# ComparativeGenomicsToolkit/cactus

Measured on NVIDIA B200. Metric: BAR POA DP Gcells/sec and ends/sec at 1/2/4/8 B200 vs reference CPU BAR, higher is better.
Workload: dtype int32

## Files before the change

cactus_b200/csrc/poa_cta.cuh:

```cuda
#pragma once
#include <cuda_runtime.h>
#include "poa_graph.cuh"

namespace barb200 {

__device__ int cta_excl_scan(int *a, int n, int *ws) {
    const int T = blockDim.x, tid = threadIdx.x, lane = tid & 31, warp = tid >> 5, nw = T >> 5;
    const int chunk = (n + T - 1) / T, b = min(n, tid * chunk), e = min(n, b + chunk);
    int s = 0;
    for (int i = b; i < e; ++i) s += a[i];
    int inc = s;
#pragma unroll
    for (int off = 1; off < 32; off <<= 1) { const int v = __shfl_up_sync(0xffffffffu, inc, off); if (lane >= off) inc += v; }
    __syncthreads();
    if (lane == 31) ws[warp] = inc;
    __syncthreads();
    int woff = 0, total = 0;
    for (int k = 0; k < nw; ++k) { const int v = ws[k]; if (k < warp) woff += v; total += v; }
    int run = woff + inc - s;
    for (int i = b; i < e; ++i) { const int v = a[i]; a[i] = run; run += v; }
    __syncthreads();
    return total;
}

// ... 99 lines not shown
    if (first_new + n_new > g.node_cap) { if (tid == 0) g.err = JOB_ERR_NODE_CAP; __syncthreads(); return; }
    for (int q = tid; q < L; q += T) {
        const int m = node_of[q];
        if (m >= 0) { is_new[q] = 0; continue; }
        const int nid = first_new + is_new[q];
        g.base[nid] = seq[q]; g.aln_n[nid] = 0;
        g.in_off[nid] = 0; g.in_n[nid] = 0; g.in_cap[nid] = 0; g.out_off[nid] = 0; g.out_n[nid] = 0; g.out_cap[nid] = 0;
        if (m != INT32_MIN) graph_add_aligned(g, -1 - m, nid);
        node_of[q] = nid; is_new[q] = 1;
    }
    if (tid == 0) g.node_n = first_new + n_new;
    __syncthreads();
    if (g.err) return;
    {
        int *anc = g.remain, *cnt = g.msa_rank, *new_i2n = g.tmp1;
        const int n_old = first_new;
        for (int q = tid; q < L; q += T) {
            const int v = node_of[q];
            int e = v < first_new ? g.node_to_index[v] : -1;
            for (int k = 0; k < g.aln_n[v]; ++k) { const int a = g.aln_id[v * 4 + k]; if (a < first_new) e = max(e, g.node_to_index[a]); }
            anc[q] = e;
        }
        for (int i = tid; i < n_old; i += T) cnt[i] = 0;
        __syncthreads();
        cta_incl_max_scan(anc, L, ws);
        for (int q = tid; q < L; q += T) if (node_of[q] >= first_new) atomicAdd(&cnt[max(anc[q], 0)], 1);
        __syncthreads();
        cta_excl_scan(cnt, n_old, ws);
        for (int i = tid; i < n_old; i += T) new_i2n[i + cnt[i]] = g.index_to_node[i];
        for (int q = tid; q < L; q += T) { const int v = node_of[q]; if (v >= first_new) new_i2n[max(anc[q], 0) + 1 + (v - first_new)] = v; }
        __syncthreads();
        for (int k = tid; k < first_new + n_new; k += T) { const int v = new_i2n[k]; g.index_to_node[k] = v; g.node_to_index[v] = k; }
        __syncthreads();
    }
    for (int q = tid; q <= L; q += T) {
        const int from = q == 0 ? SRC_ID : node_of[q - 1], to = q == L ? SINK_ID : node_of[q];
        const int fresh = (q > 0 && from >= first_new) || (q < L && to >= first_new);
        graph_add_edge_par(g, from, to, fresh ? 0 : 1, read_id);
    }
    __syncthreads();
}


__device__ __forceinline__ void prefetch_l2(const void *p) { asm volatile("prefetch.global.L2 [%0];" ::"l"(p)); }

__device__ int warp_backtrack_step(const RowTables &rt, const DpState &d, const PoaParams &P, const int *smat8, const uint8_t *q,
                                   int &i, int &j, int &cur_op, int &len) {
    const unsigned FULLM = 0xffffffffu;
    const int lane = threadIdx.x & 31, inf = P.inf_min, e1 = P.e1, e2 = P.e2, oe1 = P.o1 + P.e1, oe2 = P.o2 + P.e2;
    len = 1;
    const RowRec rc = rt.rec[i];
    const RowInfo ri = d.info[i];
    const int *rowi = d.planes + d.row_off[i];
    const int npre = rc.base_npre >> 8;
    const int s = smat8[8 * (rc.base_npre & 0xff) + q[j - 1]];
    int hij = inf; unsigned cij = (unsigned)E_NEG16 | (unsigned)E_NEG16 << 16;
    if (j >= ri.beg && j <= ri.end) { const int64_t o = plane_index(ri.beg, ri.end, 0, j); hij = __ldcg(rowi + o); cij = (unsigned)__ldcg(rowi + o + CPT); }
    int hk0 = inf;
    if ((cur_op & OP_F) && j - 1 - lane >= ri.beg && j - 1 - lane <= ri.end) hk0 = __ldcg(rowi + plane_index(ri.beg, ri.end, 0, j - 1 - lane));
    int pi = -1, pm = inf, ph = inf, pe1 = inf, pe2 = inf; bool m_in = false, e_in = false;
    auto probe = [&](int kb) {
        const int k = kb + lane;
        pi = -1; m_in = false; e_in = false;
        if (k >= npre) return;
        pi = k == 0 ? rc.pre0 : rt.pre_row[rc.pre_off + k];
        const RowInfo pin = d.info[pi];
        const int *prow = d.planes + d.row_off[pi];
        m_in = (cur_op & OP_M) && j - 1 >= pin.beg && j - 1 <= pin.end;
        e_in = (cur_op & OP_E) && j >= pin.beg && j <= pin.end;
        if (m_in) pm = __ldcg(prow + plane_index(pin.beg, pin.end, 0, j - 1));
        if (e_in) {
            const int64_t o = plane_index(pin.beg, pin.end, 0, j);
            ph = __ldcg(prow + o);
            const unsigned code = (unsigned)__ldcg(prow + o + CPT);
            pe1 = e_decode(ph, (int)(code & 0xffffu), inf); pe2 = e_decode(ph, (int)(code >> 16), inf);
        }
    };
    if (cur_op & OP_M) {
        for (int kb = 0; kb < npre; kb += 32) {
            probe(kb);
            const unsigned hit = __ballot_sync(FULLM, m_in && pm + s == hij);
            if (hit) { i = __shfl_sync(FULLM, pi, __ffs(hit) - 1); --j; cur_op = OP_ALL; return CMATCH; }
        }
    }
    if (cur_op & OP_E) {
        const int own_e1 = e_decode(hij, (int)(cij & 0xffffu), inf), own_e2 = e_decode(hij, (int)(cij >> 16), inf);
        for (int kb = 0; kb < npre; kb += 32) {
            if (npre > 32 || !(cur_op & OP_M)) probe(kb);
            const bool ok1 = e_in && (cur_op & OP_E1) && ((cur_op & OP_M) ? hij == pe1 : own_e1 == pe1 - e1);
            const bool ok2 = e_in && (cur_op & OP_E2) && ((cur_op & OP_M) ? hij == pe2 : own_e2 == pe2 - e2);
            const unsigned hit = __ballot_sync(FULLM, ok1 || ok2);
            if (hit) {
                const int f = __ffs(hit) - 1;
                const int nop = ok1 ? ((ph - oe1 == pe1) ? (OP_M | OP_F) : OP_E1) : ((ph - oe2 == pe2) ? (OP_M | OP_F) : OP_E2);
                cur_op = __shfl_sync(FULLM, nop, f); i = __shfl_sync(FULLM, pi, f);
                return CDEL;
            }
        }
    }
    if (cur_op & OP_F) {
        if (!(cur_op & OP_M)) return -1;
        const int avail = j - ri.beg;
        int t1_max;
        if (e1 > e2) t1_max = oe2 >= oe1 ? (oe2 - oe1) / (e1 - e2) + 1 : 0;
        else t1_max = (e1 < e2 || oe1 <= oe2) ? avail : 0;
        if (t1_max > avail) t1_max = avail;
        for (int which = 0; which < 2; ++which) {
            if (!(cur_op & (which ? OP_F2 : OP_F1))) continue;
            const int oe = which ? oe2 : oe1, e = which ? e2 : e1, tmax = which ? avail : t1_max;
            for (int t0 = 0; t0 < tmax; t0 += 32) {
                const int t = t0 + lane + 1;
                int hk = hk0;
                if (t0 > 0) { hk = inf; if (t <= avail) hk = __ldcg(rowi + plane_index(ri.beg, ri.end, 0, j - t)); }
                const unsigned hit = __ballot_sync(FULLM, t <= tmax && hk == hij + oe + (t - 1) * e);
                if (hit) { len = __ffs(hit); len += t0; j -= len; cur_op = OP_M | OP_E; return CINS; }
            }
        }
    }
    return -1;
}

__device__ void warp_backtrack(Graph &g, const RowTables &rt, DpState &d, const PoaParams &P, const int *smat8, const uint8_t *q, int L) {
    const unsigned FULLM = 0xffffffffu;
    const int lane = threadIdx.x & 31, inf = P.inf_min;
    if (lane == 0) { dp_best_cell(g, rt, d, P, L); d.fc_row = -1; d.fc_hi = -1; }
    __syncwarp();
    int i = d.best_i, j = d.best_j, cur_op = OP_ALL, nc = 0, last_op = -1;
    uint64_t *cg = d.cigar; const int cap = d.cigar_cap;
    int fail = 0;
    auto push = [&](int op, int len, int node_id, int query_id) {
        if (nc == 0 || op != CINS || last_op != CINS) {
            if (nc >= cap) { fail = JOB_ERR_CIGAR_CAP; return; }
            if (lane == 0) {
                const uint64_t n_id = (uint64_t)(int64_t)node_id, q_id = (uint64_t)(int64_t)query_id, l = (uint64_t)len;
                cg[nc] = op == CMATCH ? (n_id << 34 | q_id << 4 | (uint64_t)op) : op == CINS ? (q_id << 34 | l << 4 | (uint64_t)op) : (n_id << 34 | l << 4 | (uint64_t)op);
            }
            ++nc;
        } else if (lane == 0) cg[nc - 1] += (uint64_t)len << 4;
        last_op = op;
    };
    if (j < L) push(CINS, L - j, -1, L - 1);
#ifdef BT_PROFILE
    long long pf_t0 = clock64(), pf_run_t = 0, pf_step_t = 0; int pf_iters = 0, pf_runs = 0, pf_cells = 0, pf_steps = 0, pf_ins = 0;
#endif
    while (i > 0 && j > 0 && !fail) {
        int run = 0;
#ifdef BT_PROFILE
        long long pf_a = clock64();
#endif
        if (cur_op == OP_ALL) {
            int c = i - lane, pre = -1, base = 0, n_ok = 0, node = 0;
            RowInfo ric; ric.beg = 0; ric.end = -1; ric.left = 0; ric.right = 0;
            int64_t ro = 0;
            bool fresh = true;
#pragma unroll 1
            for (int it = 0; it < 4; ++it) {
                if (fresh) {
                    pre = -1;
                    if (c > 0) { const RowRec rc = rt.rec[c]; base = rc.base_npre & 0xff; pre = (rc.base_npre >> 8) ? rc.pre0 : -1; node = g.index_to_node[c]; }
                    if (c >= 0) { ric = d.info[c]; ro = d.row_off[c]; }
                }
                const int nxt = __shfl_down_sync(FULLM, c, 1);
                const bool ok = lane < 31 && pre >= 0 && pre == nxt;
                n_ok = __ffs(~__ballot_sync(FULLM, ok)) - 1;
                if (n_ok >= 31 || it == 3) break;
                const int pre_b = __shfl_sync(FULLM, pre, n_ok);
                if (pre_b < 0) break;
                fresh = lane > n_ok;
                if (fresh) c = pre_b - (lane - n_ok - 1);
            }
            const int jj = j - lane;
            int hv = inf, inb = 0;
            if (lane <= n_ok && c >= 0 && jj >= 0) {
                inb = jj >= ric.beg && jj <= ric.end;
                if (inb) hv = __ldcg(d.planes + ro + plane_index(ric.beg, ric.end, 0, jj));
            }
            const int cl = c - 32, jl = jj - 32;
            RowInfo ril; ril.beg = 0; ril.end = -1; ril.left = 0; ril.right = 0;
            int64_t rol = 0;
            if (cl >= 0 && jl >= 0) { ril = d.info[cl]; rol = d.row_off[cl]; prefetch_l2(rt.rec + cl); prefetch_l2(g.index_to_node + cl); }
            const int h_next = __shfl_down_sync(FULLM, hv, 1), inb_next = __shfl_down_sync(FULLM, inb, 1);
            bool hit = false;
            if (lane < n_ok && c > 0 && jj >= 1 && inb_next) hit = h_next + smat8[8 * base + q[jj - 1]] == hv;
            run = __ffs(~__ballot_sync(FULLM, hit)) - 1;
            if (run > 0) {
                if (nc + run > cap) fail = JOB_ERR_CIGAR_CAP;
                else {
                    if (lane < run) cg[nc + lane] = (uint64_t)node << 34 | (uint64_t)(jj - 1) << 4 | (uint64_t)CMATCH;
                    nc += run; last_op = CMATCH;
                    i = __shfl_sync(FULLM, c, run); j -= run;
                }
            }
            if (cl >= 0 && jl >= 0 && jl <= ril.end) prefetch_l2(d.planes + rol + plane_index(ril.beg, ril.end, 0, jl < ril.beg ? ril.beg : jl));
        }
#ifdef BT_PROFILE
        long long pf_b = clock64(); if (cur_op == OP_ALL) { pf_run_t += pf_b - pf_a; ++pf_iters; if (run) { ++pf_runs; pf_cells += run; } }
#endif
        if (run == 0 && !fail) {
            const int id = g.index_to_node[i], jq = j - 1;
            int len = 1;
            const int op = warp_backtrack_step(rt, d, P, smat8, q, i, j, cur_op, len);
            if (op < 0) fail = JOB_ERR_BACKTRACK; else push(op, len, id, jq);
#ifdef BT_PROFILE
            pf_step_t += clock64() - pf_b; ++pf_steps; if (op == CINS) ++pf_ins;
#endif
        }
    }
#ifdef BT_PROFILE
    if (lane == 0 && blockIdx.x == 0) printf("bt L=%d total=%lld run_t=%lld step_t=%lld iters=%d runs=%d cells=%d steps=%d ins=%d\n", L, clock64() - pf_t0, pf_run_t, pf_step_t, pf_iters, pf_runs, pf_cells, pf_steps, pf_ins);
#endif
    if (!fail && j > 0) push(CINS, j, -1, j - 1);
    if (fail) { if (lane == 0) g.err = fail; return; }
// ... 173 lines not shown
```

cactus_b200/csrc/poa_graph.cuh:

```cuda
#pragma once
#include <stdio.h>
#include "poa_types.h"

namespace barb200 {

HD void graph_reset(Graph &g, int n_seq) {
    g.node_n = 2; g.W = 1 + ((n_seq - 1) >> 6);
    g.in_used = 0; g.out_used = 0; g.err = JOB_OK;
    for (int i = 0; i < 2; ++i) {
        g.base[i] = 0; g.aln_n[i] = 0;
        g.in_off[i] = 0; g.in_n[i] = 0; g.in_cap[i] = 0;
        g.out_off[i] = 0; g.out_n[i] = 0; g.out_cap[i] = 0;
    }
}

HD int graph_add_node(Graph &g, uint8_t b) {
    if (g.node_n >= g.node_cap) { g.err = JOB_ERR_NODE_CAP; return g.node_cap - 1; }
    int id = g.node_n++;
    g.base[id] = b; g.aln_n[id] = 0;
    g.in_off[id] = 0; g.in_n[id] = 0; g.in_cap[id] = 0;
    g.out_off[id] = 0; g.out_n[id] = 0; g.out_cap[id] = 0;
    return id;
}

// ... 81 lines not shown
    g.err = JOB_ERR_TOPO;
}

HD void graph_sort_node_edges(Graph &g, int v) {
    {
        const int o = g.in_off[v], n = g.in_n[v];
        for (int j = 0; j < n - 1; ++j) for (int k = j + 1; k < n; ++k)
            if (g.in_w[o + j] < g.in_w[o + k]) {
                int t = g.in_id[o + j]; g.in_id[o + j] = g.in_id[o + k]; g.in_id[o + k] = t;
                t = g.in_w[o + j]; g.in_w[o + j] = g.in_w[o + k]; g.in_w[o + k] = t;
            }
    }
    {
        const int o = g.out_off[v], n = g.out_n[v], W = g.W;
        for (int j = 0; j < n - 1; ++j) for (int k = j + 1; k < n; ++k)
            if (g.out_w[o + j] < g.out_w[o + k]) {
                int t = g.out_id[o + j]; g.out_id[o + j] = g.out_id[o + k]; g.out_id[o + k] = t;
                t = g.out_w[o + j]; g.out_w[o + j] = g.out_w[o + k]; g.out_w[o + k] = t;
                for (int w = 0; w < W; ++w) {
                    uint64_t r = g.out_rid[(int64_t)(o + j) * W + w];
                    g.out_rid[(int64_t)(o + j) * W + w] = g.out_rid[(int64_t)(o + k) * W + w];
                    g.out_rid[(int64_t)(o + k) * W + w] = r;
                }
            }
    }
}

HD void graph_bfs_remain(Graph &g) {
    const int n = g.node_n;
    int *outdeg = g.tmp0, *q = g.tmp1;
    for (int i = 0; i < n; ++i) { outdeg[i] = g.out_n[i]; g.remain[i] = 0; }
    int head = 0, tail = 0;
    q[tail++] = SINK_ID; g.remain[SINK_ID] = -1;
    while (head < tail) {
        const int cur = q[head++];
        if (cur != SINK_ID) {
            int max_w = -1, max_id = -1;
            const int oo = g.out_off[cur], on = g.out_n[cur];
            for (int i = 0; i < on; ++i) if (g.out_w[oo + i] > max_w) { max_w = g.out_w[oo + i]; max_id = g.out_id[oo + i]; }
            g.remain[cur] = g.remain[max_id] + 1;
        }
        if (cur == SRC_ID) return;
        const int io = g.in_off[cur], in = g.in_n[cur];
        for (int i = 0; i < in; ++i) if (--outdeg[g.in_id[io + i]] == 0) q[tail++] = g.in_id[io + i];
    }
    g.err = JOB_ERR_TOPO;
}

HD void graph_build_row(const Graph &g, RowTables &rt, int r, int off) {
    const int v = g.index_to_node[r];
    const int io = g.in_off[v], in = g.in_n[v];
    for (int k = 0; k < in; ++k) rt.pre_row[off + k] = g.node_to_index[g.in_id[io + k]];
    RowRec rec;
    rec.base_npre = g.base[v] | (in << 8);
    rec.rd = g.remain[v] - g.remain[SINK_ID] - 1;
    rec.pre_off = off;
    rec.pre0 = in ? g.node_to_index[g.in_id[io]] : -1;
    rt.rec[r] = rec;
}
HD void graph_build_rows(const Graph &g, RowTables &rt) {
    int off = 0;
    for (int r = 0; r < g.node_n; ++r) { graph_build_row(g, rt, r, off); off += g.in_n[g.index_to_node[r]]; }
}
HD int row_npre(const RowTables &rt, int r) { return rt.rec[r].base_npre >> 8; }
HD int row_base(const RowTables &rt, int r) { return rt.rec[r].base_npre & 0xff; }

HD void graph_topo_sort_serial(Graph &g, RowTables &rt) {
    graph_bfs_index(g);
    if (g.err) return;
    for (int v = 0; v < g.node_n; ++v) graph_sort_node_edges(g, v);
    graph_bfs_remain(g);
    if (g.err) return;
    graph_build_rows(g, rt);
}

HD void graph_add_first_sequence(Graph &g, const uint8_t *seq, int len, int read_id) {
    int last = SRC_ID;
    for (int i = 0; i < len; ++i) { int cur = graph_add_node(g, seq[i]); graph_add_edge(g, last, cur, 0, read_id); last = cur; if (g.err) return; }
    graph_add_edge(g, last, SINK_ID, 0, read_id);
}

HD void graph_fuse_alignment(Graph &g, const uint8_t *seq, const uint64_t *cigar, int n_cigar, int read_id) {
    if (n_cigar == 0) return;
    int query_id = -1, last_new = 0, last_id = SRC_ID;
    for (int i = 0; i < n_cigar && !g.err; ++i) {
        const int op = (int)(cigar[i] & 0xf);
        if (op == CMATCH) {
            const int node_id = (int)((cigar[i] >> 34) & 0x3fffffff);
            ++query_id;
            const uint8_t b = seq[query_id];
            if (g.base[node_id] != b) {
                int a = graph_aligned_with_base(g, node_id, b);
                if (a != -1) { graph_add_edge(g, last_id, a, 1 - last_new, read_id); last_id = a; last_new = 0; }
                else {
                    int nid = graph_add_node(g, b);
                    graph_add_edge(g, last_id, nid, 0, read_id);
                    last_id = nid; last_new = 1;
                    graph_add_aligned(g, node_id, nid);
                }
            } else { graph_add_edge(g, last_id, node_id, 1 - last_new, read_id); last_id = node_id; last_new = 0; }
        } else if (op == CINS) {
            const int len = (int)((cigar[i] >> 4) & 0x3fffffff);
            query_id += len;
            for (int j = len - 1; j >= 0 && !g.err; --j) {
                int nid = graph_add_node(g, seq[query_id - j]);
                graph_add_edge(g, last_id, nid, 0, read_id);
                last_id = nid; last_new = 1;
            }
        }
    }
    if (!g.err) graph_add_edge(g, last_id, SINK_ID, 1 - last_new, read_id);
}

HD int graph_msa_rank(Graph &g) {
    const int n = g.node_n;
    int *indeg = g.tmp0, *st = g.tmp1;
    for (int i = 0; i < n; ++i) indeg[i] = g.in_n[i];
    int sp = 0, rank = 0;
// ... 250 lines not shown
```

cactus_b200/csrc/poa_kernel.cu:

```cuda
#include <cuda_runtime.h>
#include <stdint.h>
#include "poa_graph.cuh"
#include "poa_cta.cuh"
#include "poa_kernel.cuh"

namespace barb200 {

#define FULL 0xffffffffu

struct KShared {
    Graph g; RowTables rt; DpState d;
    int job, msa_len_s, abort_s;
    int smat[5 * 8];
    int wF[2][2][32];
    int wM[2][4][32];
};

__device__ __forceinline__ int4 ld4cg(const int *p) { return __ldcg(reinterpret_cast<const int4 *>(p)); }
__device__ __forceinline__ void st4(int *p, int a, int b, int c, int d) { *reinterpret_cast<int4 *>(p) = make_int4(a, b, c, d); }
__device__ __forceinline__ int max3(int a, int b, int c) { return max(max(a, b), c); }
__device__ __forceinline__ void st8(int *p, int a0, int a1, int a2, int a3, int a4, int a5, int a6, int a7) {
    asm volatile("st.global.v8.b32 [%0], {%1,%2,%3,%4,%5,%6,%7,%8};" ::"l"(p), "r"(a0), "r"(a1), "r"(a2), "r"(a3), "r"(a4), "r"(a5), "r"(a6), "r"(a7) : "memory");
}
struct int8v { int v[8]; };
__device__ __forceinline__ int8v ld8cg(const int *p) {
    int8v r;
    asm volatile("ld.global.cg.v8.b32 {%0,%1,%2,%3,%4,%5,%6,%7}, [%8];" : "=r"(r.v[0]), "=r"(r.v[1]), "=r"(r.v[2]), "=r"(r.v[3]), "=r"(r.v[4]), "=r"(r.v[5]), "=r"(r.v[6]), "=r"(r.v[7]) : "l"(p) : "memory");
    return r;
}


template <bool MASKED>
__device__ __forceinline__ void row_pass1(int (&H)[CPT], int (&E1)[CPT], int (&E2)[CPT], const int *mrow, const uint32_t (&qc)[2],
                                          int j0, int beg, int end, int NEG, int je1, int je2, int e1, int e2, int &agg1, int &agg2) {
#pragma unroll
    for (int e = 0; e < CPT; ++e) {
        const int s = mrow[(qc[e >> 3] >> ((e & 7) * 4)) & 7];
        int h = __vimax3_s32(H[e] + s, E1[e], E2[e]);
        if (MASKED) {
            const bool inb = (unsigned)(j0 + e - beg) <= (unsigned)(end - beg);
            h = inb ? h : NEG; E1[e] = inb ? E1[e] : NEG; E2[e] = inb ? E2[e] : NEG;
        }
        H[e] = h;
        agg1 = __viaddmax_s32(h, je1 + e * e1, agg1); agg2 = __viaddmax_s32(h, je2 + e * e2, agg2);
    }
}

template <int MODE>
__device__ __forceinline__ void row_pass2(int (&H)[CPT], int (&E1)[CPT], int (&E2)[CPT], int P1, int P2, int j0, int beg, int end, int NEG,
                                          int je1, int je2, int e1, int e2, int o1, int o2, int *tp, int &tmax) {
    const int oe1 = o1 + e1, oe2 = o2 + e2;
#pragma unroll
    for (int oc = 0; oc < 2; ++oc) {
        int dd[8];
#pragma unroll
        for (int u = 0; u < 8; ++u) {
            const int e = oc * 8 + u, u1 = je1 + e * e1, u2 = je2 + e * e2;
            const int f1 = P1 - o1 - u1, f2 = P2 - o2 - u2;
            P1 = __viaddmax_s32(H[e], u1, P1); P2 = __viaddmax_s32(H[e], u2, P2);
            int h = __vimax3_s32(H[e], f1, f2);
            int x1 = __viaddmax_s32(E1[e], -e1, h - oe1);
            int x2 = __viaddmax_s32(E2[e], -e2, h - oe2);
            if (MODE == 1) {
                const bool inb = (unsigned)(j0 + e - beg) <= (unsigned)(end - beg);
                h = inb ? h : NEG; x1 = inb ? x1 : NEG; x2 = inb ? x2 : NEG;
            } else if (MODE == 2) {
                const bool inb = j0 + e <= end;
                h = inb ? h : NEG; x1 = inb ? x1 : NEG; x2 = inb ? x2 : NEG;
            }
            H[e] = h; E1[e] = x1; E2[e] = x2;
            dd[u] = (h - x1) | ((h - x2) << 16);
            tmax = max(tmax, h);
        }
        st8(tp + CPT + oc * 8, dd[0], dd[1], dd[2], dd[3], dd[4], dd[5], dd[6], dd[7]);
    }
#pragma unroll
    for (int oc = 0; oc < 2; ++oc)
        st8(tp + oc * 8, H[oc * 8], H[oc * 8 + 1], H[oc * 8 + 2], H[oc * 8 + 3], H[oc * 8 + 4], H[oc * 8 + 5], H[oc * 8 + 6], H[oc * 8 + 7]);
}

template <bool MASKED>
__device__ __forceinline__ void row_argmax(const int (&H)[CPT], int v, int j0, int beg, int end, int &tl, int &tr) {
    unsigned m = 0;
#pragma unroll
    for (int e = 0; e < CPT; ++e) m |= H[e] == v ? 1u << e : 0u;
    if (MASKED) {
        const int lo = max(beg - j0, 0), hi = min(end - j0, CPT - 1);
        m &= (2u << hi) - (1u << lo);
    }
    if (m) { tl = j0 + __ffs(m) - 1; tr = j0 + 31 - __clz(m); }
}

__device__ long long dp_sweep(KShared &S, const BatchArgs &A, const uint8_t *__restrict__ qg, int L) {
    const int tid = threadIdx.x, lane = tid & 31, warp = tid >> 5, nwarps = blockDim.x >> 5;
    const PoaParams &P = A.P;
    uint8_t *const sb = A.slots + (int64_t)blockIdx.x * A.lay.slot_bytes;
    const RowRec *const rec_tab = reinterpret_cast<const RowRec *>(sb + A.lay.o_row_rec);
    const int *const pre_row = reinterpret_cast<const int *>(sb + A.lay.o_pre_row);
    RowInfo *const info = reinterpret_cast<RowInfo *>(sb + A.lay.o_row_info);
    int64_t *const row_off = reinterpret_cast<int64_t *>(sb + A.lay.o_row_off);
    int *const planes = A.planes + (int64_t)blockIdx.x * A.lay.plane_cap;
    const int64_t plane_cap = A.lay.plane_cap;
    const int node_n = S.g.node_n, R = node_n - 1;
    const int NEG = P.inf_min, e1 = P.e1, e2 = P.e2, oe1 = P.o1 + P.e1, oe2 = P.o2 + P.e2;
    const int w = P.wb + (int)(P.wf * L);
    const int pn_shift = reference_lane_count(P, L, node_n) == 16 ? 4 : 3;
    static_assert(CPT == 16, "shifts below assume 16 columns per thread");
    const int j0 = tid * CPT, je1 = j0 * e1, je2 = j0 * e2;

    uint32_t qc[2] = {0u, 0u};
#pragma unroll
    for (int e = 0; e < CPT; ++e) {
        const int j = j0 + e;
        const uint32_t c = (j >= 1 && j <= L) ? qg[j - 1] : 5u;
        qc[e >> 3] |= c << ((e & 7) * 4);
    }

    int H[CPT], E1[CPT], E2[CPT];
    bool prev_active;
    int prev_beg = 0, prev_end, prev_left = 0, prev_right = 0;
    int cur_blk = 0, cells = 0;

    {
        const int dd = L - rec_tab[0].rd;
        prev_end = min(L, max(0, dd) + w);
        const int nT = prev_end / CPT + 1;
        if ((int64_t)nT * TB > plane_cap) return -1;
        prev_active = tid < nT;
        if (prev_active) {
            int *tp = planes + tid * TB;
            int dd[CPT];
#pragma unroll
            for (int e = 0; e < CPT; ++e) {
                const int j = j0 + e;
                if (j == 0) { H[e] = 0; E1[e] = -oe1; E2[e] = -oe2; dd[e] = oe1 | (oe2 << 16); }
                else if (j <= prev_end) { H[e] = max(-P.o1 - e1 * j, -P.o2 - e2 * j); E1[e] = NEG; E2[e] = NEG; dd[e] = E_NEG16 | (E_NEG16 << 16); }
                else { H[e] = E1[e] = E2[e] = NEG; dd[e] = 0; }
            }
#pragma unroll
            for (int oc = 0; oc < 2; ++oc) {
                st8(tp + oc * 8, H[oc * 8], H[oc * 8 + 1], H[oc * 8 + 2], H[oc * 8 + 3], H[oc * 8 + 4], H[oc * 8 + 5], H[oc * 8 + 6], H[oc * 8 + 7]);
                st8(tp + CPT + oc * 8, dd[oc * 8], dd[oc * 8 + 1], dd[oc * 8 + 2], dd[oc * 8 + 3], dd[oc * 8 + 4], dd[oc * 8 + 5], dd[oc * 8 + 6], dd[oc * 8 + 7]);
            }
        } else {
#pragma unroll
            for (int e = 0; e < CPT; ++e) H[e] = E1[e] = E2[e] = NEG;
        }
        if (lane == 31) S.wM[0][3][warp] = prev_active ? H[CPT - 1] : NEG;
        if (tid == 0) { RowInfo ri; ri.beg = 0; ri.end = prev_end; ri.left = 0; ri.right = 0; info[0] = ri; row_off[0] = 0; }
        cur_blk = nT; cells = prev_end + 1;
    }
    __syncthreads();

    RowRec rec = rec_tab[R > 1 ? 1 : 0];
    for (int r = 1; r < R; ++r) {
        const int par = r & 1;
        const RowRec nrec = rec_tab[r + 1 < R ? r + 1 : r];
        const int b = rec.base_npre & 0xff, npre = rec.base_npre >> 8;
        const int dd = L - rec.rd;
        int maxL = node_n, maxR = 0, min_pre_beg = 0x7fffffff;
        bool has_prev = false;
        if (npre == 1 && rec.pre0 == r - 1) {
            maxL = min(node_n, prev_left + 1); maxR = prev_right + 1; min_pre_beg = prev_beg; has_prev = true;
        } else {
#pragma unroll 1
            for (int k = 0; k < npre; ++k) {
                const int p = k == 0 ? rec.pre0 : pre_row[rec.pre_off + k];
                int pl, pr, pb;
                if (p == r - 1) { pl = prev_left; pr = prev_right; pb = prev_beg; has_prev = true; }
                else { const RowInfo pi = info[p]; pl = pi.left; pr = pi.right; pb = pi.beg; }
                maxL = min(maxL, pl + 1); maxR = max(maxR, pr + 1); min_pre_beg = min(min_pre_beg, pb);
            }
        }
        const bool only_prev = npre == 1 && has_prev;
        int beg = max(0, min(maxL, dd) - w);
        const int end = min(L, max(maxR, dd) + w);
        if ((beg >> pn_shift) < (min_pre_beg >> pn_shift)) beg = min_pre_beg;
        const int t0 = beg >> 4, nT = (end >> 4) - t0 + 1, tt = tid - t0;
        if ((int64_t)(cur_blk + nT) * TB > plane_cap) return -1;
        const bool active = tt >= 0 && tt < nT;
        const int wmode = __any_sync(FULL, active && j0 < beg) ? 1 : __any_sync(FULL, active && j0 + CPT - 1 > end) ? 2 : 0;
        const int *mrow = S.smat + 8 * b;

        int hl = __shfl_up_sync(FULL, prev_active ? H[CPT - 1] : NEG, 1);
        if (lane == 0) hl = warp > 0 ? S.wM[par ^ 1][3][warp - 1] : NEG;

        const int id1 = NEG + beg * e1 + P.o1, id2 = NEG + beg * e2 + P.o2;
        int agg1 = id1, agg2 = id2;
        if (active) {
            if (has_prev && prev_active) {
#pragma unroll
                for (int e = CPT - 1; e >= 1; --e) H[e] = H[e - 1];
                H[0] = hl;
            } else {
#pragma unroll
                for (int e = 0; e < CPT; ++e) { H[e] = NEG; E1[e] = NEG; E2[e] = NEG; }
                if (has_prev) H[0] = hl;
            }
#pragma unroll 1
            for (int k = only_prev ? npre : 0; k < npre; ++k) {
                const int p = k == 0 ? rec.pre0 : pre_row[rec.pre_off + k];
                if (p == r - 1) continue;
                const RowInfo pi = info[p];
                const int pt0 = pi.beg >> 4, pnT = (pi.end >> 4) - pt0 + 1, ptt = tid - pt0;
                const int *Hp = planes + row_off[p] + (int64_t)ptt * TB;
                if (ptt >= 0 && ptt < pnT) {
#pragma unroll
                    for (int oc = 0; oc < 2; ++oc) {
                        const int8v h = ld8cg(Hp + oc * 8), dv = ld8cg(Hp + CPT + oc * 8);
#pragma unroll
                        for (int u = 0; u < 8; ++u) {
                            const int e = oc * 8 + u;
                            const int c1 = dv.v[u] & 0xffff, c2 = (int)((unsigned)dv.v[u] >> 16);
                            if (e + 1 < CPT) H[e + 1] = max(H[e + 1], h.v[u]);
                            E1[e] = max(E1[e], c1 == E_NEG16 ? NEG : h.v[u] - c1); E2[e] = max(E2[e], c2 == E_NEG16 ? NEG : h.v[u] - c2);
                        }
                    }
                }
                if (ptt >= 1 && ptt <= pnT) H[0] = max(H[0], __ldcg(Hp - TB + CPT - 1));
            }
            if (wmode != 1) row_pass1<false>(H, E1, E2, mrow, qc, j0, beg, end, NEG, je1, je2, e1, e2, agg1, agg2);
            else row_pass1<true>(H, E1, E2, mrow, qc, j0, beg, end, NEG, je1, je2, e1, e2, agg1, agg2);
        }
        int inc1 = agg1, inc2 = agg2;
#pragma unroll
        for (int off = 1; off < 32; off <<= 1) {
            const int n1 = __shfl_up_sync(FULL, inc1, off), n2 = __shfl_up_sync(FULL, inc2, off);
            if (lane >= off) { inc1 = max(inc1, n1); inc2 = max(inc2, n2); }
        }
        int ex1 = __shfl_up_sync(FULL, inc1, 1), ex2 = __shfl_up_sync(FULL, inc2, 1);
        if (lane == 0) { ex1 = id1; ex2 = id2; }
        if (lane == 31) { S.wF[par][0][warp] = inc1; S.wF[par][1][warp] = inc2; }
        __syncthreads();
        int P1, P2;
        {
            const int wv1 = lane < warp ? S.wF[par][0][lane] : id1, wv2 = lane < warp ? S.wF[par][1][lane] : id2;
            P1 = max(__reduce_max_sync(FULL, wv1), ex1); P2 = max(__reduce_max_sync(FULL, wv2), ex2);
        }
        int tmax = NEG - 1000;
        if (active) {
            int *tp = planes + (int64_t)(cur_blk + tt) * TB;
            if (wmode == 0) row_pass2<0>(H, E1, E2, P1, P2, j0, beg, end, NEG, je1, je2, e1, e2, P.o1, P.o2, tp, tmax);
            else if (wmode == 2) row_pass2<2>(H, E1, E2, P1, P2, j0, beg, end, NEG, je1, je2, e1, e2, P.o1, P.o2, tp, tmax);
            else row_pass2<1>(H, E1, E2, P1, P2, j0, beg, end, NEG, je1, je2, e1, e2, P.o1, P.o2, tp, tmax);
        }
        {
            const int wmax = __reduce_max_sync(FULL, tmax);
            int tleft = 0x7fffffff, tright = -1;
            if (active && tmax == wmax) {
                if (wmode == 0) row_argmax<false>(H, wmax, j0, beg, end, tleft, tright); else row_argmax<true>(H, wmax, j0, beg, end, tleft, tright);
            }
            const int wl = __reduce_min_sync(FULL, tleft), wr = __reduce_max_sync(FULL, tright);
            if (lane == 0) { S.wM[par][0][warp] = wmax; S.wM[par][1][warp] = wl; S.wM[par][2][warp] = wr; }
            if (lane == 31) S.wM[par][3][warp] = active ? H[CPT - 1] : NEG;
        }
        __syncthreads();
        {
            const int v = lane < nwarps ? S.wM[par][0][lane] : NEG - 1000;
            const int bmax = __reduce_max_sync(FULL, v);
            const int l = (lane < nwarps && v == bmax) ? S.wM[par][1][lane] : 0x7fffffff;
            const int rr = (lane < nwarps && v == bmax) ? S.wM[par][2][lane] : -1;
            prev_left = __reduce_min_sync(FULL, l); prev_right = __reduce_max_sync(FULL, rr);
        }
        prev_beg = beg; prev_end = end; prev_active = active;
        if (tid == 0) { RowInfo ri; ri.beg = beg; ri.end = end; ri.left = prev_left; ri.right = prev_right; info[r] = ri; row_off[r] = (int64_t)cur_blk * TB; }
        cur_blk += nT; cells += end - beg + 1;
        rec = nrec;
    }
    __syncthreads();
    return cells;
}

__device__ __forceinline__ void carve(KShared &S, const BatchArgs &A, int slot) {
    const SlotLayout &Y = A.lay;
    uint8_t *b = A.slots + (int64_t)slot * Y.slot_bytes;
    Graph &g = S.g; RowTables &rt = S.rt; DpState &d = S.d;
    g.node_cap = Y.node_cap; g.in_pool = Y.in_pool; g.out_pool = Y.out_pool;
    g.base = b + Y.o_base; g.aln_n = b + Y.o_aln_n; g.aln_id = (int *)(b + Y.o_aln_id);
    g.in_off = (int *)(b + Y.o_in_off); g.in_n = (int *)(b + Y.o_in_n); g.in_cap = (int *)(b + Y.o_in_cap);
    g.out_off = (int *)(b + Y.o_out_off); g.out_n = (int *)(b + Y.o_out_n); g.out_cap = (int *)(b + Y.o_out_cap);
    g.in_id = (int *)(b + Y.o_in_id); g.in_w = (int *)(b + Y.o_in_w);
    g.out_id = (int *)(b + Y.o_out_id); g.out_w = (int *)(b + Y.o_out_w); g.out_rid = (uint64_t *)(b + Y.o_out_rid);
    g.index_to_node = (int *)(b + Y.o_index_to_node); g.node_to_index = (int *)(b + Y.o_node_to_index);
    g.remain = (int *)(b + Y.o_remain); g.msa_rank = (int *)(b + Y.o_msa_rank);
    g.tmp0 = (int *)(b + Y.o_tmp0); g.tmp1 = (int *)(b + Y.o_tmp1);
    rt.rec = (RowRec *)(b + Y.o_row_rec); rt.pre_row = (int *)(b + Y.o_pre_row);
    d.planes = A.planes + (int64_t)slot * Y.plane_cap; d.plane_cap = Y.plane_cap;
    d.row_off = (int64_t *)(b + Y.o_row_off); d.info = (RowInfo *)(b + Y.o_row_info);
    d.cigar = (uint64_t *)(b + Y.o_cigar); d.cigar_cap = Y.cigar_cap; d.n_cigar = 0;
    d.fc = (int *)(b + Y.o_fc); d.fc_cap = Y.fc_cap; d.fc_row = -1; d.fc_hi = -1;
}

#define PHASE_TICK(ph) do { if (A.phase_clk && threadIdx.x == 0) { unsigned long long _n = clock64(); A.phase_clk[(size_t)blockIdx.x * PH_N + (ph)] += _n - t_last; t_last = _n; } } while (0)

__device__ __forceinline__ void poa_msa_body(const BatchArgs &A) {
    extern __shared__ __align__(16) unsigned char dyn_smem[];
    __shared__ KShared S;
    const int tid = threadIdx.x;
    int *ws = &S.wF[0][0][0];
    if (tid == 0) carve(S, A, blockIdx.x);
    for (int k = tid; k < 40; k += blockDim.x) S.smat[k] = (k & 7) < 5 ? A.P.mat[(k >> 3) * 5 + (k & 7)] : 0;
    unsigned long long t_last = A.phase_clk ? clock64() : 0ULL, t_start = t_last;
    __syncthreads();

    while (true) {
        if (tid == 0) {
            const int k = atomicAdd(A.next_job, 1);
            int j = -1;
            if (k < A.n_jobs) j = A.job_base + k;
            S.job = j;
        }
        __syncthreads();
        const int job = S.job;
        if (job < 0) break;
        const JobDesc jd = A.jobs[job];
        const int K = jd.n_seq;
        const int *lens = A.lens + jd.len_off;
        const int64_t *soff = A.soff + jd.len_off;
        const uint8_t *seqs = A.seqs + jd.seq_off;
        if (tid == 0) { graph_reset(S.g, K); S.abort_s = 0; }
        __syncthreads();
        const int *const order = A.order + jd.len_off;
        if (tid == 0 && A.gt_status[job]) S.g.err = JOB_ERR_GT_CAP;
        __syncthreads();
        long long cells = 0;
        for (int a = 0; a < K && !S.g.err; ++a) {
            const int read = order[a], L = lens[read];
            const uint8_t *q = seqs + soff[read];
            if (a == 0) {
                if (A.serial_phases) { if (tid == 0) graph_add_first_sequence(S.g, q, L, read); }
                else cta_add_first_sequence(S.g, q, L, read);
                PHASE_TICK(PH_FUSE);
            } else {
                long long c = -2;
                if (L + 1 <= CPT * (int)blockDim.x) c = dp_sweep(S, A, q, L);
                if (c < 0) { if (tid == 0) S.g.err = c == -2 ? JOB_ERR_QUERY_LEN : JOB_ERR_PLANE_CAP; c = 0; }
                cells += c;
                __syncthreads();
                PHASE_TICK(PH_DP);
                if (A.serial_phases) { if (tid == 0 && !S.g.err) { dp_best_cell(S.g, S.rt, S.d, A.P, L); dp_backtrack(S.g, S.rt, S.d, A.P, q, L); } }
                else if (tid < 32 && !S.g.err) warp_backtrack(S.g, S.rt, S.d, A.P, S.smat, q, L);
                PHASE_TICK(PH_BACKTRACK);
                __syncthreads();
                if (A.serial_phases) { if (tid == 0 && !S.g.err) graph_fuse_alignment(S.g, q, S.d.cigar, S.d.n_cigar, read); }
                else if (!S.g.err) cta_fuse_alignment(S.g, q, L, S.d.cigar, S.d.n_cigar, read, ws);
                PHASE_TICK(PH_FUSE);
            }
            __syncthreads();
            if (S.g.err) break;
            if (A.serial_phases) { if (tid == 0) graph_topo_sort_serial(S.g, S.rt); __syncthreads(); }
            else cta_topo_sort(S.g, S.rt, dyn_smem, A.scratch_bytes, ws, A.bfs_order == 0);
            PHASE_TICK(PH_TOPO);
            if (S.g.err) break;
        }
        __syncthreads();
        if (!S.g.err) {
            if (A.serial_phases) { if (tid == 0) S.msa_len_s = graph_msa_rank(S.g); __syncthreads(); }
            else cta_msa_rank(S.g, dyn_smem, A.scratch_bytes, ws, &S.msa_len_s);
            if (tid == 0 && !S.g.err && S.msa_len_s > jd.msa_stride) S.g.err = JOB_ERR_MSA_CAP;
        }
        __syncthreads();
        if (!S.g.err) {
            const int ml = S.msa_len_s;
            uint8_t *msa = A.msa + jd.msa_off;
            for (int64_t i = tid; i < (int64_t)K * ml; i += blockDim.x) msa[(i / ml) * jd.msa_stride + (i % ml)] = GAP_CODE;
            __syncthreads();
            for (int v = 2 + tid; v < S.g.node_n; v += blockDim.x) graph_msa_fill_node(S.g, v, msa, jd.msa_stride);
        }
        __syncthreads();
        if (tid == 0) { A.status[job] = S.g.err; A.msa_len[job] = S.g.err ? 0 : S.msa_len_s; A.cells[job] = cells; }
        PHASE_TICK(PH_MSA);
        __syncthreads();
    }
    if (A.phase_clk && tid == 0) A.phase_clk[(size_t)blockIdx.x * PH_N + PH_TOTAL] += clock64() - t_start;
}

extern "C" __global__ void __launch_bounds__(32, 16) poa_msa_kernel_t32(const BatchArgs A) { poa_msa_body(A); }
extern "C" __global__ void __launch_bounds__(64, 8) poa_msa_kernel_t64(const BatchArgs A) { poa_msa_body(A); }
#ifndef BARB200_T128_MINB
#define BARB200_T128_MINB 4
#endif
extern "C" __global__ void __launch_bounds__(128, BARB200_T128_MINB) poa_msa_kernel_t128(const BatchArgs A) { poa_msa_body(A); }
extern "C" __global__ void __launch_bounds__(256, 2) poa_msa_kernel_t256(const BatchArgs A) { poa_msa_body(A); }
extern "C" __global__ void __launch_bounds__(640, 1) poa_msa_kernel_t640(const BatchArgs A) { poa_msa_body(A); }
extern "C" __global__ void __launch_bounds__(1024, 1) poa_msa_kernel_t1024(const BatchArgs A) { poa_msa_body(A); }

}
```

cactus_b200/csrc/poa_types.h:

```cpp
#pragma once
#include <stdint.h>

#if defined(__CUDACC__)
#define HD __host__ __device__ __forceinline__
#else
#define HD inline
#endif

namespace barb200 {

constexpr int SRC_ID = 0;
constexpr int SINK_ID = 1;
constexpr int GAP_CODE = 5;

constexpr int OP_M = 0x1, OP_E1 = 0x2, OP_E2 = 0x4, OP_E = 0x6, OP_F1 = 0x8, OP_F2 = 0x10, OP_F = 0x18, OP_ALL = 0x1f;
constexpr int CMATCH = 0, CINS = 1, CDEL = 2;

enum JobStatus : int {
    JOB_OK = 0,
    JOB_ERR_NODE_CAP = 1,
    JOB_ERR_EDGE_CAP = 2,
    JOB_ERR_PLANE_CAP = 3,
    JOB_ERR_CIGAR_CAP = 4,
    JOB_ERR_MSA_CAP = 5,
    JOB_ERR_TOPO = 6,
    JOB_ERR_BACKTRACK = 7,
    JOB_ERR_ALIGNED_CAP = 8,
    JOB_ERR_QUERY_LEN = 9,
    JOB_ERR_GT_CAP = 10
};

struct PoaParams {
    int mat[25];
    int o1, e1, o2, e2;
    int wb; float wf;
    int max_mat, min_mis;
    int inf_min;
};

struct JobDesc {
    int n_seq;
    int64_t seq_off;
    int64_t len_off;
    int64_t msa_off;
    int msa_stride;
    int progressive;
};

struct Graph {
    int node_n, node_cap;
    int W;
    int in_used, in_pool, out_used, out_pool;
    int err;
    uint8_t *base;
    uint8_t *aln_n;
    int *aln_id;
    int *in_off, *in_n, *in_cap;
    int *out_off, *out_n, *out_cap;
    int *in_id, *in_w;
    int *out_id, *out_w;
    uint64_t *out_rid;
    int *index_to_node, *node_to_index;
    int *remain;
    int *msa_rank;
    int *tmp0, *tmp1;
};

struct alignas(16) RowRec {
    int base_npre;
    int rd;
    int pre_off;
    int pre0;
};
struct RowTables {
    RowRec *rec;
    int *pre_row;
};

struct alignas(16) RowInfo {
    int beg, end;
    int left, right;
};

constexpr int CPT = 16;
constexpr int E_NEG16 = 0xffff;
struct DpState {
    int *planes; int64_t plane_cap;
    int64_t *row_off;
    RowInfo *info;
    uint64_t *cigar; int n_cigar, cigar_cap;
    int best_i, best_j, best_score;
    int *fc;
    int fc_cap, fc_row, fc_hi;
};

constexpr int TB = 2 * CPT;
HD int64_t plane_index(int beg, int end, int plane, int j) {
    (void)end;
    return (int64_t)(j / CPT - beg / CPT) * TB + plane * CPT + j % CPT;
}
HD int64_t row_ints(int beg, int end) { return (int64_t)TB * (end / CPT - beg / CPT + 1); }
HD int e_decode(int h, int code, int inf_min) { return code == E_NEG16 ? inf_min : h - code; }
HD int e_encode(int h, int e) { const int d = h - e; return (d >= 0 && d < E_NEG16) ? d : E_NEG16; }

HD int imax(int a, int b) { return a > b ? a : b; }
HD int imin(int a, int b) { return a < b ? a : b; }

}
```

Before: 261.8.

## Cache recent DP rows in shared-memory ring and inline second-predecessor offsets

Adds a two-slot shared-memory ring holding each thread's H and packed E codes for the last two rows, so a row whose non-adjacent predecessor is r-2 reads it from shared memory instead of global planes. It also caches RowInfo and row offsets for the last eight rows in shared memory, and packs the second predecessor's distance into spare bits of the row record to avoid a pre_row lookup. The cost is extra shared-memory stores every row, a dependence on dynamic scratch size, and templating the body on thread count. The ring path skips the E_NEG16 sentinel check, which may be unsafe for rows with absent E values.

Result: slower. 256.0 (median of 6 runs) (-2.2%).

```diff
diff --git a/cactus_b200/csrc/poa_cta.cuh b/cactus_b200/csrc/poa_cta.cuh
--- a/cactus_b200/csrc/poa_cta.cuh
+++ b/cactus_b200/csrc/poa_cta.cuh
@@ -175,8 +175,8 @@
     const RowRec rc = rt.rec[i];
     const RowInfo ri = d.info[i];
     const int *rowi = d.planes + d.row_off[i];
-    const int npre = rc.base_npre >> 8;
-    const int s = smat8[8 * (rc.base_npre & 0xff) + q[j - 1]];
+    const int npre = rec_npre(rc);
+    const int s = smat8[8 * rec_base(rc) + q[j - 1]];
     int hij = inf; unsigned cij = (unsigned)E_NEG16 | (unsigned)E_NEG16 << 16;
     if (j >= ri.beg && j <= ri.end) { const int64_t o = plane_index(ri.beg, ri.end, 0, j); hij = __ldcg(rowi + o); cij = (unsigned)__ldcg(rowi + o + CPT); }
     int hk0 = inf;
@@ -280,7 +280,7 @@
             for (int it = 0; it < 4; ++it) {
                 if (fresh) {
                     pre = -1;
-                    if (c > 0) { const RowRec rc = rt.rec[c]; base = rc.base_npre & 0xff; pre = (rc.base_npre >> 8) ? rc.pre0 : -1; node = g.index_to_node[c]; }
+                    if (c > 0) { const RowRec rc = rt.rec[c]; base = rec_base(rc); pre = rec_npre(rc) ? rc.pre0 : -1; node = g.index_to_node[c]; }
                     if (c >= 0) { ric = d.info[c]; ro = d.row_off[c]; }
                 }
                 const int nxt = __shfl_down_sync(FULLM, c, 1);
diff --git a/cactus_b200/csrc/poa_graph.cuh b/cactus_b200/csrc/poa_graph.cuh
--- a/cactus_b200/csrc/poa_graph.cuh
+++ b/cactus_b200/csrc/poa_graph.cuh
@@ -157,7 +157,7 @@
     const int io = g.in_off[v], in = g.in_n[v];
     for (int k = 0; k < in; ++k) rt.pre_row[off + k] = g.node_to_index[g.in_id[io + k]];
     RowRec rec;
-    rec.base_npre = g.base[v] | (in << 8);
+    rec.base_npre = rec_pack(g.base[v], in, in > 1 ? r - g.node_to_index[g.in_id[io + 1]] : 0);
     rec.rd = g.remain[v] - g.remain[SINK_ID] - 1;
     rec.pre_off = off;
     rec.pre0 = in ? g.node_to_index[g.in_id[io]] : -1;
@@ -167,8 +167,8 @@
     int off = 0;
     for (int r = 0; r < g.node_n; ++r) { graph_build_row(g, rt, r, off); off += g.in_n[g.index_to_node[r]]; }
 }
-HD int row_npre(const RowTables &rt, int r) { return rt.rec[r].base_npre >> 8; }
-HD int row_base(const RowTables &rt, int r) { return rt.rec[r].base_npre & 0xff; }
+HD int row_npre(const RowTables &rt, int r) { return rec_npre(rt.rec[r]); }
+HD int row_base(const RowTables &rt, int r) { return rec_base(rt.rec[r]); }
 
 HD void graph_topo_sort_serial(Graph &g, RowTables &rt) {
     graph_bfs_index(g);
diff --git a/cactus_b200/csrc/poa_kernel.cu b/cactus_b200/csrc/poa_kernel.cu
--- a/cactus_b200/csrc/poa_kernel.cu
+++ b/cactus_b200/csrc/poa_kernel.cu
@@ -14,6 +14,8 @@
     int smat[5 * 8];
     int wF[2][2][32];
     int wM[2][4][32];
+    RowInfo rinfo[8];
+    int64_t roff[8];
 };
 
 __device__ __forceinline__ int4 ld4cg(const int *p) { return __ldcg(reinterpret_cast<const int4 *>(p)); }
@@ -27,6 +29,14 @@
     int8v r;
     asm volatile("ld.global.cg.v8.b32 {%0,%1,%2,%3,%4,%5,%6,%7}, [%8];" : "=r"(r.v[0]), "=r"(r.v[1]), "=r"(r.v[2]), "=r"(r.v[3]), "=r"(r.v[4]), "=r"(r.v[5]), "=r"(r.v[6]), "=r"(r.v[7]) : "l"(p) : "memory");
     return r;
+}
+
+template <bool ANY_ROW>
+__device__ __forceinline__ void pred_cell(int (&H)[CPT], int (&E1)[CPT], int (&E2)[CPT], int e, int h, int dv, int NEG) {
+    const int c1 = dv & 0xffff, c2 = (int)((unsigned)dv >> 16);
+    if (e + 1 < CPT) H[e + 1] = max(H[e + 1], h);
+    if (ANY_ROW) { E1[e] = max(E1[e], c1 == E_NEG16 ? NEG : h - c1); E2[e] = max(E2[e], c2 == E_NEG16 ? NEG : h - c2); }
+    else { E1[e] = max(E1[e], h - c1); E2[e] = max(E2[e], h - c2); }
 }
 
 
@@ -48,7 +58,7 @@
 
 template <int MODE>
 __device__ __forceinline__ void row_pass2(int (&H)[CPT], int (&E1)[CPT], int (&E2)[CPT], int P1, int P2, int j0, int beg, int end, int NEG,
-                                          int je1, int je2, int e1, int e2, int o1, int o2, int *tp, int &tmax) {
+                                          int je1, int je2, int e1, int e2, int o1, int o2, int *tp, int4 *rw, int T, int &tmax) {
     const int oe1 = o1 + e1, oe2 = o2 + e2;
 #pragma unroll
     for (int oc = 0; oc < 2; ++oc) {
@@ -73,10 +83,15 @@
             tmax = max(tmax, h);
         }
         st8(tp + CPT + oc * 8, dd[0], dd[1], dd[2], dd[3], dd[4], dd[5], dd[6], dd[7]);
+        if (rw) { rw[(4 + 2 * oc) * T] = make_int4(dd[0], dd[1], dd[2], dd[3]); rw[(5 + 2 * oc) * T] = make_int4(dd[4], dd[5], dd[6], dd[7]); }
     }
 #pragma unroll
     for (int oc = 0; oc < 2; ++oc)
         st8(tp + oc * 8, H[oc * 8], H[oc * 8 + 1], H[oc * 8 + 2], H[oc * 8 + 3], H[oc * 8 + 4], H[oc * 8 + 5], H[oc * 8 + 6], H[oc * 8 + 7]);
+    if (rw) {
+#pragma unroll
+        for (int c = 0; c < 4; ++c) rw[c * T] = make_int4(H[4 * c], H[4 * c + 1], H[4 * c + 2], H[4 * c + 3]);
+    }
 }
 
 template <bool MASKED>
@@ -91,6 +106,7 @@
     if (m) { tl = j0 + __ffs(m) - 1; tr = j0 + 31 - __clz(m); }
 }
 
+template <int T>
 __device__ long long dp_sweep(KShared &S, const BatchArgs &A, const uint8_t *__restrict__ qg, int L) {
     const int tid = threadIdx.x, lane = tid & 31, warp = tid >> 5, nwarps = blockDim.x >> 5;
     const PoaParams &P = A.P;
@@ -107,6 +123,8 @@
     const int pn_shift = reference_lane_count(P, L, node_n) == 16 ? 4 : 3;
     static_assert(CPT == 16, "shifts below assume 16 columns per thread");
     const int j0 = tid * CPT, je1 = j0 * e1, je2 = j0 * e2;
+    extern __shared__ __align__(16) unsigned char dyn_smem[];
+    int4 *const ring = A.scratch_bytes >= 2 * T * 128 ? reinterpret_cast<int4 *>(dyn_smem) : nullptr;
 
     uint32_t qc[2] = {0u, 0u};
 #pragma unroll
@@ -147,7 +165,7 @@
             for (int e = 0; e < CPT; ++e) H[e] = E1[e] = E2[e] = NEG;
         }
         if (lane == 31) S.wM[0][3][warp] = prev_active ? H[CPT - 1] : NEG;
-        if (tid == 0) { RowInfo ri; ri.beg = 0; ri.end = prev_end; ri.left = 0; ri.right = 0; info[0] = ri; row_off[0] = 0; }
+        if (tid == 0) { RowInfo ri; ri.beg = 0; ri.end = prev_end; ri.left = 0; ri.right = 0; info[0] = ri; row_off[0] = 0; S.rinfo[0] = ri; S.roff[0] = 0; }
         cur_blk = nT; cells = prev_end + 1;
     }
     __syncthreads();
@@ -156,7 +174,7 @@
     for (int r = 1; r < R; ++r) {
         const int par = r & 1;
         const RowRec nrec = rec_tab[r + 1 < R ? r + 1 : r];
-        const int b = rec.base_npre & 0xff, npre = rec.base_npre >> 8;
+        const int b = rec_base(rec), npre = rec_npre(rec);
         const int dd = L - rec.rd;
         int maxL = node_n, maxR = 0, min_pre_beg = 0x7fffffff;
         bool has_prev = false;
@@ -165,10 +183,10 @@
         } else {
 #pragma unroll 1
             for (int k = 0; k < npre; ++k) {
-                const int p = k == 0 ? rec.pre0 : pre_row[rec.pre_off + k];
+                const int p = rec_pre(rec, pre_row, r, k);
                 int pl, pr, pb;
                 if (p == r - 1) { pl = prev_left; pr = prev_right; pb = prev_beg; has_prev = true; }
-                else { const RowInfo pi = info[p]; pl = pi.left; pr = pi.right; pb = pi.beg; }
+                else { const RowInfo pi = p >= r - 8 ? S.rinfo[p & 7] : info[p]; pl = pi.left; pr = pi.right; pb = pi.beg; }
                 maxL = min(maxL, pl + 1); maxR = max(maxR, pr + 1); min_pre_beg = min(min_pre_beg, pb);
             }
         }
@@ -199,25 +217,34 @@
             }
 #pragma unroll 1
             for (int k = only_prev ? npre : 0; k < npre; ++k) {
-                const int p = k == 0 ? rec.pre0 : pre_row[rec.pre_off + k];
+                const int p = rec_pre(rec, pre_row, r, k);
                 if (p == r - 1) continue;
-                const RowInfo pi = info[p];
+                const bool near = p >= r - 8;
+                const RowInfo pi = near ? S.rinfo[p & 7] : info[p];
                 const int pt0 = pi.beg >> 4, pnT = (pi.end >> 4) - pt0 + 1, ptt = tid - pt0;
-                const int *Hp = planes + row_off[p] + (int64_t)ptt * TB;
-                if (ptt >= 0 && ptt < pnT) {
-#pragma unroll
-                    for (int oc = 0; oc < 2; ++oc) {
-                        const int8v h = ld8cg(Hp + oc * 8), dv = ld8cg(Hp + CPT + oc * 8);
-#pragma unroll
-                        for (int u = 0; u < 8; ++u) {
-                            const int e = oc * 8 + u;
-                            const int c1 = dv.v[u] & 0xffff, c2 = (int)((unsigned)dv.v[u] >> 16);
-                            if (e + 1 < CPT) H[e + 1] = max(H[e + 1], h.v[u]);
-                            E1[e] = max(E1[e], c1 == E_NEG16 ? NEG : h.v[u] - c1); E2[e] = max(E2[e], c2 == E_NEG16 ? NEG : h.v[u] - c2);
+                if (ring && p == r - 2 && p > 0) {
+                    const int4 *rb = ring + par * 8 * T + tid;
+                    if (ptt >= 0 && ptt < pnT) {
+#pragma unroll
+                        for (int c = 0; c < 4; ++c) {
+                            const int4 h = rb[c * T], dv = rb[(4 + c) * T];
+                            pred_cell<false>(H, E1, E2, 4 * c, h.x, dv.x, NEG); pred_cell<false>(H, E1, E2, 4 * c + 1, h.y, dv.y, NEG);
+                            pred_cell<false>(H, E1, E2, 4 * c + 2, h.z, dv.z, NEG); pred_cell<false>(H, E1, E2, 4 * c + 3, h.w, dv.w, NEG);
                         }
                     }
+                    if (ptt >= 1 && ptt <= pnT) H[0] = max(H[0], rb[3 * T - 1].w);
+                } else {
+                    const int *Hp = planes + (near ? S.roff[p & 7] : row_off[p]) + (int64_t)ptt * TB;
+                    if (ptt >= 0 && ptt < pnT) {
+#pragma unroll
+                        for (int oc = 0; oc < 2; ++oc) {
+                            const int8v h = ld8cg(Hp + oc * 8), dv = ld8cg(Hp + CPT + oc * 8);
+#pragma unroll
+                            for (int u = 0; u < 8; ++u) pred_cell<true>(H, E1, E2, oc * 8 + u, h.v[u], dv.v[u], NEG);
+                        }
+                    }
+                    if (ptt >= 1 && ptt <= pnT) H[0] = max(H[0], __ldcg(Hp - TB + CPT - 1));
                 }
-                if (ptt >= 1 && ptt <= pnT) H[0] = max(H[0], __ldcg(Hp - TB + CPT - 1));
             }
             if (wmode != 1) row_pass1<false>(H, E1, E2, mrow, qc, j0, beg, end, NEG, je1, je2, e1, e2, agg1, agg2);
             else row_pass1<true>(H, E1, E2, mrow, qc, j0, beg, end, NEG, je1, je2, e1, e2, agg1, agg2);
@@ -240,9 +267,10 @@
         int tmax = NEG - 1000;
         if (active) {
             int *tp = planes + (int64_t)(cur_blk + tt) * TB;
-            if (wmode == 0) row_pass2<0>(H, E1, E2, P1, P2, j0, beg, end, NEG, je1, je2, e1, e2, P.o1, P.o2, tp, tmax);
-            else if (wmode == 2) row_pass2<2>(H, E1, E2, P1, P2, j0, beg, end, NEG, je1, je2, e1, e2, P.o1, P.o2, tp, tmax);
-            else row_pass2<1>(H, E1, E2, P1, P2, j0, beg, end, NEG, je1, je2, e1, e2, P.o1, P.o2, tp, tmax);
+            int4 *rw = ring ? ring + par * 8 * T + tid : nullptr;
+            if (wmode == 0) row_pass2<0>(H, E1, E2, P1, P2, j0, beg, end, NEG, je1, je2, e1, e2, P.o1, P.o2, tp, rw, T, tmax);
+            else if (wmode == 2) row_pass2<2>(H, E1, E2, P1, P2, j0, beg, end, NEG, je1, je2, e1, e2, P.o1, P.o2, tp, rw, T, tmax);
+            else row_pass2<1>(H, E1, E2, P1, P2, j0, beg, end, NEG, je1, je2, e1, e2, P.o1, P.o2, tp, rw, T, tmax);
         }
         {
             const int wmax = __reduce_max_sync(FULL, tmax);
@@ -263,7 +291,10 @@
             prev_left = __reduce_min_sync(FULL, l); prev_right = __reduce_max_sync(FULL, rr);
         }
         prev_beg = beg; prev_end = end; prev_active = active;
-        if (tid == 0) { RowInfo ri; ri.beg = beg; ri.end = end; ri.left = prev_left; ri.right = prev_right; info[r] = ri; row_off[r] = (int64_t)cur_blk * TB; }
+        if (tid == 0) {
+            RowInfo ri; ri.beg = beg; ri.end = end; ri.left = prev_left; ri.right = prev_right;
+            info[r] = ri; row_off[r] = (int64_t)cur_blk * TB; S.rinfo[r & 7] = ri; S.roff[r & 7] = (int64_t)cur_blk * TB;
+        }
         cur_blk += nT; cells += end - beg + 1;
         rec = nrec;
     }
@@ -293,6 +324,7 @@
 
 #define PHASE_TICK(ph) do { if (A.phase_clk && threadIdx.x == 0) { unsigned long long _n = clock64(); A.phase_clk[(size_t)blockIdx.x * PH_N + (ph)] += _n - t_last; t_last = _n; } } while (0)
 
+template <int T>
 __device__ __forceinline__ void poa_msa_body(const BatchArgs &A) {
     extern __shared__ __align__(16) unsigned char dyn_smem[];
     __shared__ KShared S;
@@ -333,7 +365,7 @@
                 PHASE_TICK(PH_FUSE);
             } else {
                 long long c = -2;
-                if (L + 1 <= CPT * (int)blockDim.x) c = dp_sweep(S, A, q, L);
+                if (L + 1 <= CPT * (int)blockDim.x) c = dp_sweep<T>(S, A, q, L);
                 if (c < 0) { if (tid == 0) S.g.err = c == -2 ? JOB_ERR_QUERY_LEN : JOB_ERR_PLANE_CAP; c = 0; }
                 cells += c;
                 __syncthreads();
@@ -375,14 +407,14 @@
     if (A.phase_clk && tid == 0) A.phase_clk[(size_t)blockIdx.x * PH_N + PH_TOTAL] += clock64() - t_start;
 }
 
-extern "C" __global__ void __launch_bounds__(32, 16) poa_msa_kernel_t32(const BatchArgs A) { poa_msa_body(A); }
-extern "C" __global__ void __launch_bounds__(64, 8) poa_msa_kernel_t64(const BatchArgs A) { poa_msa_body(A); }
+extern "C" __global__ void __launch_bounds__(32, 16) poa_msa_kernel_t32(const BatchArgs A) { poa_msa_body<32>(A); }
+extern "C" __global__ void __launch_bounds__(64, 8) poa_msa_kernel_t64(const BatchArgs A) { poa_msa_body<64>(A); }
 #ifndef BARB200_T128_MINB
 #define BARB200_T128_MINB 4
 #endif
-extern "C" __global__ void __launch_bounds__(128, BARB200_T128_MINB) poa_msa_kernel_t128(const BatchArgs A) { poa_msa_body(A); }
-extern "C" __global__ void __launch_bounds__(256, 2) poa_msa_kernel_t256(const BatchArgs A) { poa_msa_body(A); }
-extern "C" __global__ void __launch_bounds__(640, 1) poa_msa_kernel_t640(const BatchArgs A) { poa_msa_body(A); }
-extern "C" __global__ void __launch_bounds__(1024, 1) poa_msa_kernel_t1024(const BatchArgs A) { poa_msa_body(A); }
-
-}
+extern "C" __global__ void __launch_bounds__(128, BARB200_T128_MINB) poa_msa_kernel_t128(const BatchArgs A) { poa_msa_body<128>(A); }
+extern "C" __global__ void __launch_bounds__(256, 2) poa_msa_kernel_t256(const BatchArgs A) { poa_msa_body<256>(A); }
+extern "C" __global__ void __launch_bounds__(640, 1) poa_msa_kernel_t640(const BatchArgs A) { poa_msa_body<640>(A); }
+extern "C" __global__ void __launch_bounds__(1024, 1) poa_msa_kernel_t1024(const BatchArgs A) { poa_msa_body<1024>(A); }
+
+}
diff --git a/cactus_b200/csrc/poa_types.h b/cactus_b200/csrc/poa_types.h
--- a/cactus_b200/csrc/poa_types.h
+++ b/cactus_b200/csrc/poa_types.h
@@ -76,6 +76,14 @@
     RowRec *rec;
     int *pre_row;
 };
+HD int rec_pack(int base, int npre, int d1) { return base | ((d1 >= 1 && d1 <= 15) ? d1 << 4 : 0) | npre << 8; }
+HD int rec_base(const RowRec &c) { return c.base_npre & 0xf; }
+HD int rec_npre(const RowRec &c) { return c.base_npre >> 8; }
+HD int rec_pre(const RowRec &c, const int *pre_row, int r, int k) {
+    if (k == 0) return c.pre0;
+    const int d1 = (c.base_npre >> 4) & 0xf;
+    return (k == 1 && d1) ? r - d1 : pre_row[c.pre_off + k];
+}
 
 struct alignas(16) RowInfo {
     int beg, end;
```
